# imcbrearty/GENIE

Hardware: AMD Instinct MI355X
Metric: picks/sec through GCN_Detection_Network_extended.forward_fixed_source (GCS_Network.forward) (higher is better)
Workload: dtype f32

## Files before the change

genie_amd/csrc/genie_hip.hip:

```cpp
#include <hip/hip_runtime.h>
#include <stdint.h>
#include <stdio.h>
#include <stdlib.h>
#include <string.h>

#include <algorithm>
#include <array>
#include <map>
#include <memory>
#include <mutex>
#include <utility>
#include <type_traits>
#include <string>
#include <vector>

#include "genie_hip.h"

#define GENIE_LD_STREAM(ptr) (*(ptr))
#define GENIE_S2_WAVES 2
#define GENIE_H2_DEPTH 6

namespace {

typedef float f32x4 __attribute__((ext_vector_type(4)));

thread_local std::string g_err;

int fail(int code, const std::string& msg) {
    g_err = msg;
    return code;
}

#define HIP_TRY(expr)                                                                              \
    do {                                                                                           \
        hipError_t e_ = (expr);                                                                    \
        if (e_ != hipSuccess)                                                                      \
            return fail(GENIE_ERR_HIP, std::string(#expr) + ": " + hipGetErrorString(e_));         \
    } while (0)
#define GENIE_TRY(expr)                                                                            \
    do {                                                                                           \
        if (int rc_ = (expr)) return rc_;                                                          \
    } while (0)

struct DevPool {
    std::multimap<size_t, void*> free_;
    size_t cached = 0;
};
std::map<int, DevPool> g_pools;
std::map<void*, std::pair<int, size_t>> g_pool_blocks;
std::mutex g_pool_mutex;
constexpr size_t POOL_CAP = (size_t)3 << 30;

size_t pool_class(size_t n) {
    if (n < 256) return 256;
    int sh = 0;
    while ((n >> sh) >= 16) ++sh;
    const size_t step = (size_t)1 << sh;
    return (n + step - 1) / step * step;
}

hipError_t gmalloc(void** p, size_t bytes) {
    int dev = 0;
    hipError_t e = hipGetDevice(&dev);
    if (e != hipSuccess) return e;
    const size_t cls = pool_class(bytes);
    {
        std::lock_guard<std::mutex> lk(g_pool_mutex);
        DevPool& P = g_pools[dev];
        auto it = P.free_.find(cls);
        if (it != P.free_.end()) {
            *p = it->second;
            P.cached -= cls;
            P.free_.erase(it);
            return hipSuccess;
        }
    }
    e = hipMalloc(p, cls);
    if (e != hipSuccess) {
        std::lock_guard<std::mutex> lk(g_pool_mutex);
        DevPool& P = g_pools[dev];
        (void)hipDeviceSynchronize();
        for (auto& kv : P.free_) { g_pool_blocks.erase(kv.second); (void)hipFree(kv.second); }
        P.free_.clear(); P.cached = 0;
        e = hipMalloc(p, cls);
        if (e != hipSuccess) return e;
    }
    std::lock_guard<std::mutex> lk(g_pool_mutex);
    g_pool_blocks[*p] = std::make_pair(dev, cls);
    return hipSuccess;
}
template <typename T> hipError_t gmalloc(T** p, size_t bytes) { return gmalloc((void**)p, bytes); }

hipError_t gfree(void* p) {
    if (!p) return hipSuccess;
    std::lock_guard<std::mutex> lk(g_pool_mutex);
    auto it = g_pool_blocks.find(p);
    if (it == g_pool_blocks.end()) return hipFree(p);
    DevPool& P = g_pools[it->second.first];
    const size_t cls = it->second.second;
// ... 976 lines not shown
#include "aux_kernels.hpp"
#include "train_tail_kernels.hpp"
#include "train_assoc_kernels.hpp"
#include "train_arrival_kernels.hpp"
#include "detect_kernels.hpp"
#include "stack_kernels.hpp"
#include "select_kernels.hpp"
#include "cloud_kernels.hpp"
#include "optim_kernels.hpp"
#include "pointer_kernels.hpp"

}

enum class RowLayout { Rows, NodePlanar };

struct ModelTables {
    StagePlan plan[NPLAN];
    DevBuf<StepDesc> d_steps[NPLAN];
    DevBuf<BiasDesc> d_bias[NPLAN];
    DevBuf<int32_t> d_scal[NPLAN];
    DevBuf<AccDesc> d_acc[NTM]; DevBuf<VecDesc> d_vec[NTM]; DevBuf<int32_t> d_sc[NTM];
    int n_acc[NTM] = {}, n_vec[NTM] = {}, n_sc[NTM] = {};
    DevBuf<int32_t> d_h2tbl;
    DevBuf<int32_t> d_s2htbl;
};

struct RevGraph {
    DevBuf<int32_t> rowptr, col;
    DevBuf<float> w;
    DevBuf<int2> cw;
};

struct genie_ctx {
    int S, G, G_ext, T;
    float scale_rel, scale_t;
    long long P, P_ext, E_src;
    DevBuf<int32_t> sta_rowptr, sta_col, src_rowptr, src_col, order, outdeg;
    DevBuf<float> raw;
    bool dirty;
    const ModelTables* tb;
    DevBuf<PackPlan> d_packplans; int pack_blocks;
    DevBuf<float> packed[NPLAN];
    DevBuf<float> as_pg;
    DevBuf<float> as_ps;
    RevGraph r_sta, r_src;
    RevGraph rp_sta, rp_src;
    DevBuf<int32_t> ptile16, ptile32;
    const float *xs_slice, *xs_mask;
    const void* xs_ws;
    int xs_mm_copy;
    DevBuf<float> abs_sta, abs_src;
    DevBuf<unsigned> abs_ts, abs_tg;
    bool abs_dirty;
    int abs_ts_order;
    bool pcsr;
    bool pcsr_h2;
    DevBuf<int32_t> p_sta_rowptr, p_sta_col, p_src_rowptr, p_src_col, seg_rowptr;
    DevBuf<int32_t> p_src_of;
    DevBuf<int32_t> p_sta_of;
    DevBuf<float> mpos_sta, mpos_src, ebias_sta, ebias_src;
    bool has_edges;
    DevBuf<int32_t> sta_perm, sta_inv, sta_rowptr_p, sta_col_p;
    DevBuf<int32_t> sta_ident;
    DevBuf<float> ebias_sta_p;
    const float* ea_user;
    DevBuf<int32_t> src_tab;
    DevBuf<float> packed_h2;
    hipStream_t side_stream;
    hipEvent_t ev_fork, ev_join;
    int device = 0;
    int num_cu;
    int seg, bpc1, bpc2;
    int ks_uni, kp_uni;
    int use_fast;
    int bpc2o;
    int s2_wgmap;
    int bpc1b;
    int use_h2;
    int prec_mode;
    bool range_ok;
    float range_act, range_w;
    DevBuf<float> d_range; float* h_range;
    unsigned* h_inflag;
    struct S2uTables { DevBuf<S2uBlock> blocks; DevBuf<int32_t> xcd0; int nblk; };
    std::map<std::pair<int, int>, S2uTables> s2u;
    std::vector<int32_t> tab_host;
    DevBuf<float> packed_s2h;
    DevBuf<unsigned> ea_frag, ea_frag_tmp;
    RowLayout s1_layout;
    std::vector<const void*> lds_attr_done;
    int xs_sta_order;
    int sign_input;
    int no_phase;
    int tail_f32;
    size_t o_xs, o_mm, o_c, o_wu, o_wv, o_part, o_sa0, o_sa1, o_bip, o_gpart, o_pj0, o_pj1, o_cv, ws_floats;
    size_t slot_stride;
    size_t big_stride;
    int tail_cu_ro, tail_cu_sa;
    int slot;

    ~genie_ctx() {
        if (h_range) (void)hipHostFree(h_range);
        if (h_inflag) (void)hipHostFree(h_inflag);
        if (ev_fork) (void)hipEventDestroy(ev_fork);
        if (ev_join) (void)hipEventDestroy(ev_join);
    }
};

namespace {

int raise_lds_limit(genie_ctx* c, const void* kern, int bytes) {
    for (const void* k : c->lds_attr_done) if (k == kern) return GENIE_OK;
    HIP_TRY(hipFuncSetAttribute(kern, hipFuncAttributeMaxDynamicSharedMemorySize, bytes));
    c->lds_attr_done.push_back(kern);
    return GENIE_OK;
}

long long edge_rows_sta(const genie_ctx* c) { return c->pcsr ? c->P : c->S; }
long long edge_rows_src(const genie_ctx* c) { return c->pcsr ? c->P : c->G; }
bool h2_on(const genie_ctx* c) { return c->use_h2 && (c->prec_mode == 1 || (c->prec_mode == 0 && c->range_ok)); }
bool pcsr_h2_on(const genie_ctx* c) { return c->pcsr_h2 && (c->prec_mode == 1 || (c->prec_mode == 0 && c->range_ok)); }
int part_T(const genie_ctx* c) { return c->pcsr ? 1 : c->T; }
bool abs_generic(const genie_ctx* c) { return c->abs_sta != nullptr && (c->has_edges || !h2_on(c)); }

struct StageCall {
    float* save;
    bool train;
};
constexpr StageCall kInference{nullptr, false};

bool sta_order_on(const genie_ctx* c, const StageCall& call) {
    return c->sta_perm != nullptr && !c->pcsr && h2_on(c) && !abs_generic(c) && !call.train;
}
bool tail_wide(const genie_ctx* c, const StageCall& call) { return !c->tail_f32 && !call.train; }

enum class S1Route {
    Generic,
    PcsrH2,
    PcsrF32,
    H2,
};
enum class S2Route {
    TrainAssoc,
    TrainH2u,
    TrainOrd,
    Generic,
    PcsrPseg,
    PcsrSeg,
    AssocLast,
    H2u,
};
struct StageRoutes {
    S1Route s1;
    S2Route s2;
    RowLayout layout;
};
StageRoutes stage_routes(const genie_ctx* c, const StageCall& call, int gi_begin, int gi_end, bool no_bip, bool want_xl) {
    StageRoutes r;
    if (c->pcsr) {
        r.s1 = pcsr_h2_on(c) && !(c->abs_sta && c->has_edges) ? S1Route::PcsrH2 : S1Route::PcsrF32;
        r.s2 = !no_bip && !want_xl && !call.save ? S2Route::PcsrPseg : S2Route::PcsrSeg;
    } else {
        r.s1 = h2_on(c) && !abs_generic(c) ? S1Route::H2 : S1Route::Generic;
        const bool whole = gi_begin == 0 && gi_end == c->G;
        const bool fast = c->use_fast && !abs_generic(c);
        if (call.train) {
            if (fast && no_bip && want_xl && whole) r.s2 = S2Route::TrainAssoc;
// ... 1021 lines not shown
            }
            a.abs_ts = c->abs_ts; a.abs_tg = c->abs_tg;
        }
        launch_stage1_h2<true>(a, c->abs_sta != nullptr, c->has_edges, c->P * XROW >= (1ll << 32), grid, st);
        break;
    }
    case S1Route::PcsrF32: {
        const long long ntiles = (c->P + 15) / 16;
        a.ptile = c->ptile16;
        const long long gw = std::min<long long>((ntiles + 3) / 4, (long long)c->num_cu * c->bpc1);
        k_stage1_pcsr<<<(int)std::max<long long>(8, gw / 8 * 8), 256, 0, st>>>(a);
        break;
    }
    case S1Route::H2: {
        unsigned* xs = (unsigned*)((float*)ws + c->o_xs);
        const bool presplit = (c->xs_slice == slice && c->xs_mask == mask && c->xs_ws == ws && c->xs_sta_order == (so ? 1 : 0)) || !do_split;
        if (do_split) { c->xs_slice = c->xs_mask = nullptr; c->xs_ws = nullptr; }
        float* mmw = (float*)ws + c->o_mm + (c->slot % GENIE_NBIG) * c->big_stride;
        if (presplit && do_split && so && c->xs_mm_copy != c->slot % GENIE_NBIG) {
            HIP_TRY(hipMemcpyAsync(mmw, (const float*)ws + c->o_mm + c->xs_mm_copy * c->big_stride, sizeof(float) * (size_t)c->P_ext,
                                   hipMemcpyDeviceToDevice, st));
        }
        if (!presplit) {
            if (so && c->S <= SPLIT_G_MAXS) {
                HIP_TRY(hipFuncSetAttribute((const void*)k_split_rows_g, hipFuncAttributeMaxDynamicSharedMemorySize, SPLIT_G_MAXS * 32));
                k_split_rows_g<<<(unsigned)(c->P_ext / c->S), 256, (size_t)c->S * 32, st>>>(slice, mask, c->S, xs, c->sta_perm, mmw, c->P_ext,
                                                                                            input_limit(c), c->h_inflag);
            } else
                k_split_rows<<<(unsigned)((c->P_ext + 255) / 256), 256, 0, st>>>(slice, mask, c->P_ext, xs, so ? c->sta_perm : nullptr, c->S,
                                                                                mmw, input_limit(c), c->h_inflag);
        }
        a.xs = xs; a.packed = c->packed_h2; a.xs_plane = c->P_ext * (long long)XPC;
        a.np = r.layout == RowLayout::NodePlanar ? 1 : 0;
        const int grid = da_grid_w(c, (n_tiles + 1) / 2, c->bpc1b, H2_THREADS / 64);
        if (!n_tiles) break;
        if (c->abs_sta && (c->abs_dirty || !c->abs_ts || c->abs_ts_order != (so ? 1 : 0))) {
            if (!c->abs_ts) GENIE_TRY(alloc_abs_pieces(c, (size_t)c->S, (size_t)c->G_ext));
            k_abs_pieces<<<(c->S + 255) / 256, 256, 0, st>>>(c->abs_sta, so ? c->sta_perm : nullptr, c->S, c->abs_ts);
            k_abs_pieces<<<(c->G_ext + 255) / 256, 256, 0, st>>>(c->abs_src, nullptr, c->G_ext, c->abs_tg);
            c->abs_dirty = false; c->abs_ts_order = so ? 1 : 0;
            a.abs_ts = c->abs_ts; a.abs_tg = c->abs_tg;
        }
        launch_stage1_h2<false>(a, c->abs_sta != nullptr, c->has_edges, c->P_ext * XROW >= (1ll << 32), grid, st);
        break;
    }
    }
    HIP_TRY(hipGetLastError());
    if (dbg_tmp) {
        if (dbg_h0) k_permute_sta_rows<<<(unsigned)((c->P * 30 + 255) / 256), 256, 0, st>>>(dbg_tmp, c->P, 30, c->sta_perm, c->S, dbg_h0);
        if (dbg_h1) k_permute_sta_rows<<<(unsigned)((c->P * 60 + 255) / 256), 256, 0, st>>>(dbg_tmp + c->P * 30, c->P, 60, c->sta_perm, c->S, dbg_h1);
        HIP_TRY(hipStreamSynchronize(st));
    }
    return GENIE_OK;
}
}

int genie_da_stage1(genie_ctx* c, const float* slice, const float* mask, void* ws, void* stream) {
    if (!c) return fail(GENIE_ERR_ARG, "null context");
    return run_stage1(c, kInference, slice, mask, nullptr, nullptr, ws, stream, 0, c->G, true);
}

int genie_da_stage1_range(genie_ctx* c, const float* slice, const float* mask, int gi_begin, int gi_end, int first, void* ws,
                          void* stream) {
    if (!c) return fail(GENIE_ERR_ARG, "null context");
    return run_stage1(c, kInference, slice, mask, nullptr, nullptr, ws, stream, gi_begin, gi_end, first != 0);
}

int genie_da_stage1_debug(genie_ctx* c, const float* slice, const float* mask, float* h0_out, float* h1_out, void* ws,
                          void* stream) {
    if (!c || !h0_out || !h1_out) return fail(GENIE_ERR_ARG, "genie_da_stage1_debug: null argument");
    return run_stage1(c, kInference, slice, mask, h0_out, h1_out, ws, stream, 0, c->G, true);
}

float* genie_ws_v_ptr(const genie_ctx* c, void* ws) {
    return (c && ws) ? (float*)ws + c->o_wv + (c->slot % GENIE_NBIG) * c->big_stride : nullptr;
}
int genie_ws_v_pitch(const genie_ctx* c) { (void)c; return ROWW; }

namespace {
int get_s2u_tables(genie_ctx* c, int gb0, int ge0, const genie_ctx::S2uTables** out) {
    const auto key = std::make_pair(gb0, ge0);
    auto itf = c->s2u.find(key);
    if (itf != c->s2u.end()) { *out = &itf->second; return GENIE_OK; }
    const std::vector<int32_t>& tab = c->tab_host;
    std::vector<S2uBlock> blks;
    std::vector<int32_t> seen_blk((size_t)c->G_ext, -1), seen_at((size_t)c->G_ext, 0);
    int32_t serial = 0;
    int32_t x0[9];
    const int nxc = 8, n = ge0 - gb0;
    for (int x = 0; x < nxc; ++x) {
        x0[x] = (int32_t)blks.size();
        const int gb = gb0 + (int)((long long)n * x / nxc), ge = gb0 + (int)((long long)n * (x + 1) / nxc);
        int pos = gb;
        while (pos < ge) {
            S2uBlock b;
            memset(&b, 0, sizeof(b));
            b.gi0 = pos;
            ++serial;
            int32_t uni[S2U_UCAP + 15];
            int nuni = 0;
            while (pos < ge && b.n < S2U_NB) {
                int32_t where[15];
                const int before = nuni;
                for (int k = 0; k < 15; ++k) {
                    const int32_t nb = tab[(size_t)pos * 16 + 1 + k];
                    if (seen_blk[(size_t)nb] != serial) { seen_blk[(size_t)nb] = serial; seen_at[(size_t)nb] = nuni; uni[nuni++] = nb; }
                    where[k] = seen_at[(size_t)nb];
                }
                if (b.n > 0 && nuni > S2U_UCAP) {
                    for (int u = before; u < nuni; ++u) seen_blk[(size_t)uni[u]] = -1;
                    nuni = before;
                    break;
                }
                b.idx[b.n][0] = tab[(size_t)pos * 16];
                for (int k = 0; k < 15; ++k) b.idx[b.n][1 + k] = where[k];
                ++b.n; ++pos;
            }
            for (int e = b.n; e < S2U_NB; ++e) b.idx[e][0] = -1;
            b.U = (int32_t)nuni;
            for (int u = 0; u < 64; ++u) b.ids[u] = uni[u < nuni ? u : 0];
            blks.push_back(b);
        }
    }
    x0[nxc] = (int32_t)blks.size();
    genie_ctx::S2uTables t;
    t.nblk = (int)blks.size();
    GENIE_TRY(dev_upload(t.blocks, blks));
    GENIE_TRY(dev_upload(t.xcd0, x0, (size_t)nxc + 1));
    *out = &(c->s2u[key] = std::move(t));
    return GENIE_OK;
}

extern "C++" template <bool SAVE>
int launch_stage2_h2u(genie_ctx* c, const DaArgs& a, int gi_begin, int gi_end, bool xl, hipStream_t st) {
    const genie_ctx::S2uTables* tb = nullptr;
    if (int rc = get_s2u_tables(c, gi_begin, gi_end, &tb)) return rc;
    const size_t lds = sizeof(float) * S2H_IMG_FLOATS + (size_t)S2U_UCAP * 1024;
    const long long items = (long long)tb->nblk * c->T;
    const int grid = (int)std::max<long long>(8, std::min<long long>((long long)c->num_cu * GENIE_S2U_BPC, (items + 7) / 8 * 8) / 8 * 8);
    const bool big = c->P_ext * 128 >= (1ll << 32);
    auto launch = [&](auto kern) -> int {
        if (int r = raise_lds_limit(c, (const void*)kern, 160 * 1024)) return r;
        kern<<<grid, S2U_WPB * 64, lds, st>>>(a, tb->blocks, tb->xcd0);
        return GENIE_OK;
    };
    if (xl) return big ? launch(k_stage2_h2u<true, true, SAVE>) : launch(k_stage2_h2u<true, false, SAVE>);
    return big ? launch(k_stage2_h2u<false, true, SAVE>) : launch(k_stage2_h2u<false, false, SAVE>);
}

int run_stage2(genie_ctx* c, const StageCall& call, const float* mask, const float* edge_attr, float* x_latent_out, void* ws,
               void* stream, int gi_begin, int gi_end, const float* slope2 = nullptr, int no_bip = 0) {
    int rc = check_ws(c, ws);
    if (rc) return rc;
    if (!mask || !edge_attr) return fail(GENIE_ERR_ARG, "genie_da_stage2_partials: null argument");
    if (gi_begin < 0 || gi_end > c->G || gi_begin > gi_end) return fail(GENIE_ERR_ARG, "genie_da_stage2_partials: bad source-node range");
    if (!(gi_begin == 0 && gi_end == c->G) && c->pcsr)
        return fail(GENIE_ERR_STATE, "genie_da_stage2_partials_range: not available on an irregular product graph");
    hipStream_t st = (hipStream_t)stream;
    if ((rc = ensure_packed(c, st))) return rc;
    DaArgs a = make_da_args(c, call, (float*)ws);
    a.gi0 = gi_begin; a.G = gi_end - gi_begin;
    a.slope2 = slope2; a.no_bip = no_bip;
    const long long n_tiles = (long long)a.G * c->T;
    if (n_tiles == 0) return GENIE_OK;
    const StageRoutes r = stage_routes(c, call, gi_begin, gi_end, no_bip != 0, x_latent_out != nullptr);
    if (!no_bip && c->s1_layout != r.layout)
        return fail(GENIE_ERR_STATE, r.layout == RowLayout::NodePlanar
                                         ? "stage 2: this call's stage 2 reads c / wv node-planar, but the last stage 1 wrote them as rows"
                                         : "stage 2: this call's stage 2 reads c / wv as rows, but the last stage 1 wrote them node-planar");
    a.mask = mask; a.edge_attr = edge_attr; a.x_latent = x_latent_out; a.packed = c->packed[PL_S2];
    a.ea_int = nullptr;
    a.mm_int = (const float*)ws + c->o_mm + (c->slot % GENIE_NBIG) * c->big_stride;
    auto identity_order = [&]() -> int {
        if (!c->sta_ident) {
            std::vector<int32_t> id((size_t)c->S);
            for (int i = 0; i < c->S; ++i) id[i] = i;
            GENIE_TRY(dev_upload(c->sta_ident, id));
        }
        a.sta_user = c->sta_ident; a.wgmap = 0;
        return GENIE_OK;
    };
    switch (r.s2) {
    case S2Route::TrainAssoc:
        if ((rc = identity_order())) return rc;
        k_stage2_ord<8, 15, true, true, true><<<da_grid(c, n_tiles, c->bpc2o), 256, 0, st>>>(a);
        break;
    case S2Route::TrainH2u:
        if ((rc = identity_order())) return rc;
        a.ea_int = edge_attr; a.np = 1; a.packed = c->packed_s2h;
        if (!c->ea_frag_tmp) HIP_TRY(c->ea_frag_tmp.alloc(8 * (size_t)c->P));
        k_ea_frag<<<(unsigned)((c->P + 255) / 256), 256, 0, st>>>(edge_attr, c->P, c->S, nullptr, c->ea_frag_tmp);
        a.ea_frag = c->ea_frag_tmp;
        if ((rc = launch_stage2_h2u<true>(c, a, gi_begin, gi_end, x_latent_out != nullptr, st))) return rc;
        break;
    case S2Route::TrainOrd:
        if ((rc = identity_order())) return rc;
        a.ea_int = edge_attr;
        if (x_latent_out) k_stage2_ord<8, 15, true, false, true><<<da_grid(c, n_tiles, c->bpc2o), 256, 0, st>>>(a);
        else k_stage2_ord<8, 15, false, false, true><<<da_grid(c, n_tiles, c->bpc2o), 256, 0, st>>>(a);
        break;
    case S2Route::Generic:
        k_stage2<<<da_grid(c, n_tiles, c->bpc2), 256, 0, st>>>(a);
        break;
    case S2Route::PcsrPseg: {
        a.ptile = c->ptile16;
        const long long gs = std::min<long long>((c->G + 3) / 4, (long long)c->num_cu * c->bpc2);
        k_stage2_pseg<<<(int)std::max<long long>(8, gs / 8 * 8), 256, 0, st>>>(a, c->seg_rowptr, c->G);
        break;
    }
    case S2Route::PcsrSeg: {
        const long long ntiles = (c->P + 15) / 16;
        a.ptile = c->ptile16;
        const long long gw = std::min<long long>((ntiles + 3) / 4, (long long)c->num_cu * c->bpc2);
        k_stage2_pcsr<<<(int)std::max<long long>(8, gw / 8 * 8), 256, 0, st>>>(a);
        if (!no_bip)
            k_seg_sum32<<<(c->G * 32 + 255) / 256, 256, 0, st>>>((const float*)ws + c->o_c + (c->slot % GENIE_NBIG) * c->big_stride, c->seg_rowptr,
                                                                 c->G, (float*)ws + c->o_part + c->slot * c->slot_stride);
        break;
    }
    case S2Route::AssocLast:
        a.wgmap = 0;
        k_stage2_ord<8, 15, true, true><<<da_grid(c, n_tiles, c->bpc2o), 256, 0, st>>>(a);
        break;
    case S2Route::H2u:
        a.wgmap = c->s2_wgmap; a.np = 1; a.packed = c->packed_s2h;
        if (c->ea_frag && c->ea_user == edge_attr) a.ea_frag = c->ea_frag;
// ... 1684 lines not shown
```

genie_amd/csrc/stage_kernels.hpp:

```cpp

template <int N>
__device__ __forceinline__ void mma_blocks(f32x4 (&acc)[N], const f32x4 (&w)[N], const f32x4 x) {
#pragma unroll
    for (int r = 0; r < 4; ++r) {
#pragma unroll
        for (int k = 0; k < N; ++k) acc[k] = MFMA16(w[k][r], x[r], acc[k]);
    }
}

__device__ __forceinline__ void stage1_dense(const DaArgs& a, const f32x4* lw, const float* lbias, int lane, int q,
                                             bool valid, long long p, int g, int sc, float mq, f32x4 x0, f32x4 x1, f32x4 n1a,
                                             f32x4 n1b, f32x4 n2a, f32x4 n2b, float a1, float a21, float a22) {
    if (a.dbg_h0 != nullptr && valid) {
#pragma unroll
        for (int r = 0; r < 4; ++r) {
            a.dbg_h0[p * 30 + 4 * q + r] = x0[r];
            if (16 + 4 * q + r < 30) a.dbg_h0[p * 30 + 16 + 4 * q + r] = x1[r];
        }
    }
    f32x4 acc[4], w4[4];
#pragma unroll
    for (int k = 0; k < 4; ++k) acc[k] = *(const f32x4*)(lbias + (2 + k) * 16 + 4 * q);
    if (a.eb_sta != nullptr) {
#pragma unroll
// ... 1233 lines not shown
            }
        for (int i = t; i < 990; i += 256) { const float x = fabsf(W(RG_FC1_W)[i]); bad |= !(x <= 3.0e38f); wmax = fmaxf(wmax, x); }
    }
    if (t < 30) {
        float z = fabsf(W(RG_INIT_B)[t]);
        for (int j = 0; j < 8; ++j) z += fabsf(W(RG_INIT_W)[t * 8 + j]);
        for (int j = 0; j < 3; ++j) z += fabsf(W(RG_INIT_ABS)[t * 6 + j]) * pos_sta + fabsf(W(RG_INIT_ABS)[t * 6 + 3 + j]) * pos_src;
        H0[t] = g1(a0) * z; N1[t] = g1(s11) * z; N2[t] = g1(s12) * z;
        amax = fmaxf(fmaxf(amax, fmaxf(pos_sta, pos_src)), fmaxf(H0[t], fmaxf(N1[t], N2[t])));
    }
    __syncthreads();
    if (t < 60) {
        const int i = t % 30, hf = t / 30;
        const float* w = W(hf ? RG_L1T22_W : RG_L1T12_W) + i * 64;
        const float* n = hf ? N2 : N1;
        float z = fabsf(W(hf ? RG_L1T22_B : RG_L1T12_B)[i]) + (hf ? ebg : ebs);
        for (int j = 0; j < 30; ++j) z += fabsf(w[j]) * H0[j] + fabsf(w[30 + j]) * n[j];
        for (int j = 0; j < 4; ++j) z += fabsf(w[60 + j]);
        (hf ? H1b : H1a)[i] = g1(a1) * z;
        amax = fmaxf(amax, g1(a1) * z);
    }
    __syncthreads();
    if (t < 60) {
        const int i = t % 30, hf = t / 30;
        const float* w = W(hf ? RG_L2T21_W : RG_L2T11_W) + i * 60;
        float z = fabsf(W(hf ? RG_L2T21_B : RG_L2T11_B)[i]);
        for (int j = 0; j < 30; ++j) z += fabsf(w[j]) * H1a[j] + fabsf(w[30 + j]) * H1b[j];
        const float s = hf ? a22 : a21;
        (hf ? V : U)[i] = g1(s) * z;
        amax = fmaxf(amax, g1(s) * z);
    }
    __syncthreads();
    if (t < 30) {
        const int i = t % 15, hf = t / 15;
        const float* w = W(hf ? RG_L2T22_W : RG_L2T12_W) + i * 94;
        const float* uv = hf ? V : U;
        float z = fabsf(W(hf ? RG_L2T22_B : RG_L2T12_B)[i]) + (hf ? ebg : ebs);
        for (int j = 0; j < 30; ++j) z += fabsf(w[j]) * H1a[j] + fabsf(w[30 + j]) * H1b[j] + fabsf(w[60 + j]) * uv[j];
        for (int j = 0; j < 4; ++j) z += fabsf(w[90 + j]);
        amax = fmaxf(amax, g1(a2) * z);
    }
    bad |= !(amax <= 3.0e38f);
    const float am = blk_max256(bad ? __builtin_inff() : amax, red);
    const float wm = blk_max256(bad ? __builtin_inff() : wmax, red);
    if (t == 0) {
        a.out[0] = am; a.out[1] = wm;
        a.out[2] = (am < H2_RANGE_LIMIT && wm < H2_RANGE_LIMIT) ? 1.f : 0.f;
        a.out[3] = 0.f;
    }
}

#define MFMA16H(a, b, c) \
    __builtin_amdgcn_mfma_f32_16x16x32_f16(__builtin_bit_cast(f16x8, (a)), __builtin_bit_cast(f16x8, (b)), (c), 0, 0, 0)

__global__ void k_ea_frag(const float* __restrict__ ea, long long rows, int S, const int32_t* __restrict__ sta_user,
                          unsigned* __restrict__ out) {
    const long long p = (long long)blockIdx.x * blockDim.x + threadIdx.x;
    if (p >= rows) return;
    const long long g = p / S;
    const int s = (int)(p - g * S);
    const long long pu = g * S + (sta_user != nullptr ? sta_user[s] : s);
    const float e0 = ea[pu * 3], e1 = ea[pu * 3 + 1], e2 = ea[pu * 3 + 2];
    const unsigned a0 = cvt_pk_f16(e0, e1), b0 = cvt_pk_f16(e2, 0.f);
    const unsigned a1 = cvt_pk_f16(sub_f16_lo(e0, a0), sub_f16_hi(e1, a0)), b1 = cvt_pk_f16(sub_f16_lo(e2, b0), 0.f);
    *(u32x4*)(out + ((g * 2) * S + s) * 4) = u32x4{a0, b0, a1, b1};
    *(u32x4*)(out + ((g * 2 + 1) * S + s) * 4) = u32x4{pk_mul_f16(a0, H2_SIXTEENTH), pk_mul_f16(b0, H2_SIXTEENTH), 0u, 0u};
}

template <bool BIG>
__device__ __forceinline__ unsigned long long s2h_base(const void* b, int id, unsigned pitch) {
    const unsigned long long off = BIG ? (unsigned long long)(unsigned)id * (unsigned long long)pitch
                                       : (unsigned long long)((unsigned)id * pitch);
    unsigned long long r = (unsigned long long)b + off;
    asm volatile("" : "+s"(r));
    return r;
}

constexpr int S2U_WPB = 4;
constexpr int S2U_NB = 2 * S2U_WPB;
#define GENIE_S2U_BPC 2
#define GENIE_S2U_UCAP 64
constexpr int S2U_UCAP = GENIE_S2U_UCAP;
constexpr int S2U_NSTG = S2U_UCAP / S2U_WPB;
struct S2uBlock {
    int32_t gi0, n, U, pad;
    int32_t ids[64];
    int32_t idx[S2U_NB][16];
};

template <bool XL, bool BIG, bool SAVE = false>
__global__ __launch_bounds__(S2U_WPB * 64, GENIE_S2U_BPC) void k_stage2_h2u(DaArgs a, const S2uBlock* __restrict__ blocks, const int32_t* __restrict__ xcd_blk0) {
    constexpr int KS = 8, KP = 15;
    constexpr int NF4 = S2H_IMG_FLOATS / 4;
    extern __shared__ __attribute__((aligned(16))) f32x4 s2u_smem[];
    f32x4* lw = s2u_smem;
    char* lrows = (char*)(s2u_smem + NF4);
    for (int i = threadIdx.x; i < NF4; i += blockDim.x) lw[i] = ((const f32x4*)a.packed)[i];
    const float* lbias = (const float*)(lw + S2H_FRAGS * 64);
    int lane = threadIdx.x & 63;
    const int m = lane & 15, kg = lane >> 4;
    const int jl = lane >> 2, ql = lane & 3;
    const int wave = __builtin_amdgcn_readfirstlane(threadIdx.x >> 6);
    const int S = a.S, T = a.T;
    const int nx = (a.nxcd > 1 && gridDim.x >= (unsigned)a.nxcd && (gridDim.x % a.nxcd) == 0) ? a.nxcd : 1;
    const int xcd = blockIdx.x % nx, lb = blockIdx.x / nx, nbx = gridDim.x / nx;
    const int blk0 = nx == 1 ? xcd_blk0[0] : xcd_blk0[xcd], blk1 = nx == 1 ? xcd_blk0[a.nxcd] : xcd_blk0[xcd + 1];
    const long long n_items = (long long)(blk1 - blk0) * T;
    __syncthreads();
    if (lb >= n_items) return;
    const float a2 = a.slope2 != nullptr ? *a.slope2 : lbias[32], ab1 = lbias[33];
    typedef const __attribute__((address_space(1))) char* gbytes;
    typedef const __attribute__((address_space(1))) f32x4* grow;
    typedef const __attribute__((address_space(1))) u32x4* gfrag;
    typedef const __attribute__((address_space(1))) float* gflt;
    const unsigned plane = (unsigned)S * 16u;
    const unsigned pc = (unsigned)S * 128u, pw = (unsigned)S * 64u, pe = (unsigned)S * 32u, pm = (unsigned)S * 4u;
    const unsigned kgp = (unsigned)kg * plane, kge = (unsigned)min(kg, 1) * plane;
    const unsigned q16 = 16u * (unsigned)ql;
    const int bperm = (4 * m + kg) * 4;
    const unsigned m_T = ItemIter::recip((unsigned)T);

    long long it_last = lb;
    while (it_last + nbx < n_items) it_last += nbx;
    auto item_of = [&](long long it, int& blk, int& tb) {
        const long long itr = n_items - 1 - (it <= it_last ? it : it_last);
        unsigned rem;
        const unsigned kb = T <= 1 ? (rem = 0u, (unsigned)itr) : ItemIter::fdiv((unsigned)itr, (unsigned)T, m_T, rem);
        blk = __builtin_amdgcn_readfirstlane(blk0 + (int)kb);
        tb = __builtin_amdgcn_readfirstlane((int)rem);
    };
    f32x4 stg[S2U_NSTG];
    auto stage_issue = [&](int idl, int U, int tb) {
        const int s = tb * 16 + m, sc = s < S ? s : S - 1;
        const unsigned lo = kgp + (unsigned)sc * 16u;
#pragma unroll
        for (int i = 0; i < S2U_NSTG; ++i) {
            const int u = wave + S2U_WPB * i;
            if (u < U) {
                const unsigned long long vb = s2h_base<BIG>(a.wv, __builtin_amdgcn_readlane(idl, u), pw);
                stg[i] = *(grow)((gbytes)vb + lo);
            }
        }
    };
    auto stage_write = [&](int U) {
#pragma unroll
        for (int i = 0; i < S2U_NSTG; ++i) {
            const int u = wave + S2U_WPB * i;
            if (u < U) *(f32x4*)(lrows + (unsigned)u * 1024u + (unsigned)lane * 16u) = stg[i];
        }
    };
    struct Node { f32x4 ru[KS], c1, c2; u32x4 ea; float mq; } R;
    int sta[KS];
    auto load_sta = [&](int tb) {
        const int s = tb * 16 + jl;
        load_sta_ids<KS>(a.sta_col, s < S ? s : S - 1, sta);
    };
    auto issue = [&](int idv, int tb) {
        const int g = max(__builtin_amdgcn_readlane(idv, 0), 0);
        const int s = tb * 16 + m, sc = s < S ? s : S - 1;
        const unsigned so = (unsigned)sc * 16u;
        const unsigned lo = kgp + so;
        const unsigned long long cb = s2h_base<BIG>(a.c, g, pc);
        R.c1 = *(grow)((gbytes)cb + lo);
        R.c2 = *(grow)((gbytes)cb + (lo + 4u * plane));
        const unsigned long long mb = s2h_base<BIG>(a.mm_int, g, pm);
        R.mq = *(gflt)((gbytes)mb + (unsigned)sc * 4u);
        if (s >= S) R.mq = 0.f;
        const unsigned long long eb = s2h_base<BIG>(a.ea_frag, g, pe);
        R.ea = *(gfrag)((gbytes)eb + (kge + so));
        const unsigned long long ub = s2h_base<BIG>(a.wu, g, pw);
#pragma unroll
        for (int k = 0; k < KS; ++k) R.ru[k] = *(grow)((gbytes)ub + ((unsigned)sta[k] * 64u + q16));
    };
    auto slot = [&](long long j, int& blk, int& tb, int& b) {
        item_of(lb + (j >> 1) * nbx, blk, tb);
        b = wave + S2U_WPB * (int)(j & 1);
    };
    auto idv_at = [&](long long j) {
        int blk, tb, b;
        slot(j, blk, tb, b);
        return blocks[blk].idx[b][m];
    };
    const long long n_my_items = (n_items - lb + nbx - 1) / nbx;
    int blk_c, tb_c, blk_n, tb_n, blk_2, tb_2, dummy;
    item_of(lb, blk_c, tb_c);
    item_of(lb + nbx, blk_n, tb_n);
    int idl_c = blocks[blk_c].ids[lane], U_c = blocks[blk_c].U;
    int idl_n = blocks[blk_n].ids[lane], U_n = blocks[blk_n].U;
    stage_issue(idl_c, __builtin_amdgcn_readfirstlane(U_c), tb_c);
    int idv_c = idv_at(0), idv_n = idv_at(1);
    load_sta(tb_c);
    issue(idv_c, tb_c);
    for (long long ii = 0; ii < n_my_items; ++ii) {
        const bool has_next_item = ii + 1 < n_my_items;
        item_of(lb + (ii + 2) * nbx, blk_2, tb_2);
        const int idl_2 = blocks[blk_2].ids[lane], U_2 = blocks[blk_2].U;
        stage_write(__builtin_amdgcn_readfirstlane(U_c));
        __syncthreads();
        if (has_next_item) stage_issue(idl_n, __builtin_amdgcn_readfirstlane(U_n), tb_n);
#pragma unroll
        for (int h = 0; h < 2; ++h) {
            asm volatile("" : "+v"(lane));
            const long long j = 2 * ii + h;
            const int idv_2 = idv_at(j + 2 < 2 * n_my_items ? j + 2 : j);
            const int g_raw = __builtin_amdgcn_readlane(idv_c, 0);
            const bool live = g_raw >= 0;
            const int g_c = max(g_raw, 0);
            const int tbc = tb_c;
            const int tb_next = h == 0 ? tb_c : tb_n;
            (void)dummy;
            f32x4 n1 = {0.f, 0.f, 0.f, 0.f}, n2 = {0.f, 0.f, 0.f, 0.f};
#pragma unroll
            for (int k = 0; k < KS; ++k) n1 += R.ru[k];
#pragma unroll
            for (int k0 = 0; k0 < KP; k0 += 5) {
                f32x4 rv[5];
#pragma unroll
                for (int k = 0; k < 5; ++k)
                    rv[k] = *(const f32x4*)(lrows + (unsigned)__builtin_amdgcn_readlane(idv_c, 1 + k0 + k) * 1024u + (unsigned)lane * 16u);
#pragma unroll
                for (int k = 0; k < 5; ++k) n2 += rv[k];
            }
            f32x4 n1t;
#pragma unroll
            for (int r = 0; r < 4; ++r) {
                const float v = n1[r];
                n1t[r] = __int_as_float(__builtin_amdgcn_ds_bpermute(bperm, __float_as_int(v)));
            }
            f32x4 o1 = fma4(n1t, 1.f / (float)KS, R.c1), o2 = fma4(n2, 1.f / (float)KP, R.c2);
            const float mq = R.mq;
            const u32x4 eab = R.ea;
            const long long p_sv = SAVE ? (long long)g_c * S + a.sta_user[min(tbc * 16 + m, S - 1)] : 0;
            const bool sv_ok = SAVE && live && tbc * 16 + m < S;
            if (sv_ok) {
                *(f32x4*)(a.save + ((size_t)(SV_O + 0) * a.Pn + p_sv) * 16 + 4 * kg) = o1;
                *(f32x4*)(a.save + ((size_t)(SV_O + 1) * a.Pn + p_sv) * 16 + 4 * kg) = o2;
            }
            o1 = prelu4u(o1, a2);
            o2 = prelu4u(o2, a2);
            asm volatile("" : "+v"(o1), "+v"(o2), "+v"(idv_n));
            issue(idv_n, tb_next);
            if (h == 0) load_sta(tb_n);
            if (XL && live && tbc * 16 + m < S) {
                const int su = a.sta_user[tbc * 16 + m];
                float* xl = a.x_latent + ((long long)g_c * S + su) * 30;
#pragma unroll
                for (int r = 0; r < 4; ++r)
                    if (4 * kg + r < 15) { xl[4 * kg + r] = o1[r]; xl[15 + 4 * kg + r] = o2[r]; }
            }
            u32x4 p0, p1, p2;
            p0[0] = cvt_pk_f16(o1[0], o1[1]); p0[1] = cvt_pk_f16(o1[2], o1[3]);
            p0[2] = cvt_pk_f16(o2[0], o2[1]); p0[3] = cvt_pk_f16(o2[2], o2[3]);
            p1[0] = cvt_pk_f16(sub_f16_lo(o1[0], p0[0]), sub_f16_hi(o1[1], p0[0]));
            p1[1] = cvt_pk_f16(sub_f16_lo(o1[2], p0[1]), sub_f16_hi(o1[3], p0[1]));
            p1[2] = cvt_pk_f16(sub_f16_lo(o2[0], p0[2]), sub_f16_hi(o2[1], p0[2]));
            p1[3] = cvt_pk_f16(sub_f16_lo(o2[2], p0[3]), sub_f16_hi(o2[3], p0[3]));
#pragma unroll
            for (int d = 0; d < 4; ++d) p2[d] = pk_mul_f16(p0[d], H2_SIXTEENTH);
            f32x4 bp[2];
#pragma unroll
            for (int t = 0; t < 2; ++t) {
                bp[t] = *(const f32x4*)(lbias + 16 * t + 4 * kg);
                const f32x4 w0 = lw[(S2H_FW + 2 * t) * 64 + lane], w1 = lw[(S2H_FW + 2 * t + 1) * 64 + lane];
                const f32x4 we = lw[(S2H_FE + t) * 64 + lane];
                bp[t] = MFMA16H(w0, p1, bp[t]);
                bp[t] = MFMA16H(w1, p2, bp[t]);
                bp[t] = MFMA16H(we, eab, bp[t]);
                bp[t] = MFMA16H(w0, p0, bp[t]);
                if (sv_ok) *(f32x4*)(a.save + ((size_t)(SV_ZB + t) * a.Pn + p_sv) * 16 + 4 * kg) = bp[t];
            }
#pragma unroll
            for (int t = 0; t < 2; ++t) {
                f32x4 v = prelu4u(bp[t], ab1) * mq;
                v.x = row_sum16_tree(v.x); v.y = row_sum16_tree(v.y); v.z = row_sum16_tree(v.z); v.w = row_sum16_tree(v.w);
                if (m == 0 && live) *(f32x4*)(a.part + ((long long)g_c * T + tbc) * 32 + 16 * t + 4 * kg) = v;
            }
            idv_c = idv_n; idv_n = idv_2;
        }
        if (!has_next_item) break;
        __syncthreads();
        blk_c = blk_n; tb_c = tb_n; blk_n = blk_2; tb_n = tb_2;
        idl_c = idl_n; U_c = U_n; idl_n = idl_2; U_n = U_2;
    }
}
```

Measured before the change: 78.41 million.

## Carry staged neighbour rows across grouped stage-2 blocks to reuse LDS

```diff
diff --git a/genie_amd/csrc/genie_hip.hip b/genie_amd/csrc/genie_hip.hip
--- a/genie_amd/csrc/genie_hip.hip
+++ b/genie_amd/csrc/genie_hip.hip
@@ -15,6 +15,7 @@
 #include <vector>
 
 #include "genie_hip.h"
+#include "s2u_plan.hpp"
 
 #define GENIE_LD_STREAM(ptr) (*(ptr))
 #define GENIE_S2_WAVES 2
@@ -1157,7 +1158,7 @@
     float range_act, range_w;
     DevBuf<float> d_range; float* h_range;
     unsigned* h_inflag;
-    struct S2uTables { DevBuf<S2uBlock> blocks; DevBuf<int32_t> xcd0; int nblk; };
+    struct S2uTables { DevBuf<S2uBlock> blocks; DevBuf<int32_t> xcd0; int nblk, ngroups; };
     std::map<std::pair<int, int>, S2uTables> s2u;
     std::vector<int32_t> tab_host;
     DevBuf<float> packed_s2h;
@@ -2345,51 +2346,15 @@
     const auto key = std::make_pair(gb0, ge0);
     auto itf = c->s2u.find(key);
     if (itf != c->s2u.end()) { *out = &itf->second; return GENIE_OK; }
-    const std::vector<int32_t>& tab = c->tab_host;
-    std::vector<S2uBlock> blks;
-    std::vector<int32_t> seen_blk((size_t)c->G_ext, -1), seen_at((size_t)c->G_ext, 0);
-    int32_t serial = 0;
-    int32_t x0[9];
-    const int nxc = 8, n = ge0 - gb0;
-    for (int x = 0; x < nxc; ++x) {
-        x0[x] = (int32_t)blks.size();
-        const int gb = gb0 + (int)((long long)n * x / nxc), ge = gb0 + (int)((long long)n * (x + 1) / nxc);
-        int pos = gb;
-        while (pos < ge) {
-            S2uBlock b;
-            memset(&b, 0, sizeof(b));
-            b.gi0 = pos;
-            ++serial;
-            int32_t uni[S2U_UCAP + 15];
-            int nuni = 0;
-            while (pos < ge && b.n < S2U_NB) {
-                int32_t where[15];
-                const int before = nuni;
-                for (int k = 0; k < 15; ++k) {
-                    const int32_t nb = tab[(size_t)pos * 16 + 1 + k];
-                    if (seen_blk[(size_t)nb] != serial) { seen_blk[(size_t)nb] = serial; seen_at[(size_t)nb] = nuni; uni[nuni++] = nb; }
-                    where[k] = seen_at[(size_t)nb];
-                }
-                if (b.n > 0 && nuni > S2U_UCAP) {
-                    for (int u = before; u < nuni; ++u) seen_blk[(size_t)uni[u]] = -1;
-                    nuni = before;
-                    break;
-                }
-                b.idx[b.n][0] = tab[(size_t)pos * 16];
-                for (int k = 0; k < 15; ++k) b.idx[b.n][1 + k] = where[k];
-                ++b.n; ++pos;
-            }
-            for (int e = b.n; e < S2U_NB; ++e) b.idx[e][0] = -1;
-            b.U = (int32_t)nuni;
-            for (int u = 0; u < 64; ++u) b.ids[u] = uni[u < nuni ? u : 0];
-            blks.push_back(b);
-        }
-    }
-    x0[nxc] = (int32_t)blks.size();
+    s2u_plan::Plan plan;
+    if (!s2u_plan::build(c->tab_host.data(), c->G, c->G_ext, gb0, ge0, S2U_GROUP, plan))
+        return fail(GENIE_ERR_ARG, "stage 2: a source-neighbour index outside the context's source nodes");
     genie_ctx::S2uTables t;
-    t.nblk = (int)blks.size();
-    GENIE_TRY(dev_upload(t.blocks, blks));
-    GENIE_TRY(dev_upload(t.xcd0, x0, (size_t)nxc + 1));
+    t.nblk = (int)plan.blocks.size();
+    t.ngroups = 0;
+    for (int x = 0; x < s2u_plan::NXCD; ++x) t.ngroups += (plan.xcd0[x + 1] - plan.xcd0[x] + S2U_GROUP - 1) / S2U_GROUP;
+    GENIE_TRY(dev_upload(t.blocks, plan.blocks));
+    GENIE_TRY(dev_upload(t.xcd0, plan.xcd0, (size_t)s2u_plan::NXCD + 1));
     *out = &(c->s2u[key] = std::move(t));
     return GENIE_OK;
 }
@@ -2399,12 +2364,14 @@
     const genie_ctx::S2uTables* tb = nullptr;
     if (int rc = get_s2u_tables(c, gi_begin, gi_end, &tb)) return rc;
     const size_t lds = sizeof(float) * S2H_IMG_FLOATS + (size_t)S2U_UCAP * 1024;
-    const long long items = (long long)tb->nblk * c->T;
+    static_assert(s2u_plan::NXCD == 8, "the grid below is a multiple of 8 workgroups, one share per chunk of the plan");
+    if (a.nxcd != s2u_plan::NXCD) return fail(GENIE_ERR_STATE, "stage 2: the block table is planned for 8 XCD chunks");
+    const long long items = (long long)tb->ngroups * c->T;
     const int grid = (int)std::max<long long>(8, std::min<long long>((long long)c->num_cu * GENIE_S2U_BPC, (items + 7) / 8 * 8) / 8 * 8);
     const bool big = c->P_ext * 128 >= (1ll << 32);
     auto launch = [&](auto kern) -> int {
         if (int r = raise_lds_limit(c, (const void*)kern, 160 * 1024)) return r;
-        kern<<<grid, S2U_WPB * 64, lds, st>>>(a, tb->blocks, tb->xcd0);
+        kern<<<grid, S2U_WPB * 64, lds, st>>>(a, tb->blocks, tb->xcd0, S2U_GROUP);
         return GENIE_OK;
     };
     if (xl) return big ? launch(k_stage2_h2u<true, true, SAVE>) : launch(k_stage2_h2u<true, false, SAVE>);
diff --git a/genie_amd/csrc/s2u_plan.hpp b/genie_amd/csrc/s2u_plan.hpp
--- /dev/null
+++ b/genie_amd/csrc/s2u_plan.hpp
@@ -0,0 +1,121 @@
+#pragma once
+#include <cstdint>
+#include <cstring>
+#include <vector>
+
+namespace s2u_plan {
+
+constexpr int NB = 8;
+constexpr int UCAP = 64;
+constexpr int KP = 15;
+constexpr int NXCD = 8;
+
+struct Block {
+    int32_t gi0, n, U, nst;
+    int32_t ids[64];
+    int32_t idx[NB][16];
+    uint8_t slot[64];
+};
+
+struct Plan {
+    std::vector<Block> blocks;
+    int32_t xcd0[NXCD + 1];
+    int L;
+    long long rows_union, rows_carried;
+    double carried_fraction() const { return rows_union ? (double)rows_carried / (double)rows_union : 0.0; }
+};
+
+inline bool build(const int32_t* tab, int n_pos, int n_nodes, int gb0, int ge0, int L, Plan& out) {
+    out.blocks.clear();
+    out.L = L;
+    out.rows_union = out.rows_carried = 0;
+    for (int x = 0; x <= NXCD; ++x) out.xcd0[x] = 0;
+    if (!tab || gb0 < 0 || ge0 > n_pos || gb0 > ge0 || L < 1 || n_nodes < 1) return false;
+    for (size_t i = (size_t)gb0 * 16; i < (size_t)ge0 * 16; ++i)
+        if ((i & 15) && (tab[i] < 0 || tab[i] >= n_nodes)) return false;
+    std::vector<int32_t> seen_blk((size_t)n_nodes, -1), seen_at((size_t)n_nodes, 0);
+    std::vector<int32_t> slot_of((size_t)n_nodes, -1);
+    int32_t serial = 0;
+    const int n = ge0 - gb0;
+    for (int x = 0; x < NXCD; ++x) {
+        out.xcd0[x] = (int32_t)out.blocks.size();
+        const int gb = gb0 + (int)((long long)n * x / NXCD), ge = gb0 + (int)((long long)n * (x + 1) / NXCD);
+        int pos = gb;
+        int32_t occ[UCAP], last_use[UCAP];
+        int in_group = 0;
+        for (int s = 0; s < UCAP; ++s) { occ[s] = -1; last_use[s] = -1; }
+        while (pos < ge) {
+            Block b;
+            memset(&b, 0, sizeof(b));
+            b.gi0 = pos;
+            ++serial;
+            int32_t uni[UCAP + KP];
+            int nuni = 0;
+            while (pos < ge && b.n < NB) {
+                int32_t where[KP];
+                const int before = nuni;
+                for (int k = 0; k < KP; ++k) {
+                    const int32_t nb = tab[(size_t)pos * 16 + 1 + k];
+                    if (seen_blk[(size_t)nb] != serial) { seen_blk[(size_t)nb] = serial; seen_at[(size_t)nb] = nuni; uni[nuni++] = nb; }
+                    where[k] = seen_at[(size_t)nb];
+                }
+                if (b.n > 0 && nuni > UCAP) {
+                    for (int u = before; u < nuni; ++u) seen_blk[(size_t)uni[u]] = -1;
+                    nuni = before;
+                    break;
+                }
+                b.idx[b.n][0] = tab[(size_t)pos * 16];
+                for (int k = 0; k < KP; ++k) b.idx[b.n][1 + k] = where[k];
+                ++b.n; ++pos;
+            }
+            if (nuni > UCAP) return false;
+            for (int e = b.n; e < NB; ++e) b.idx[e][0] = -1;
+            b.U = (int32_t)nuni;
+            int32_t slot_u[UCAP];
+            int nst = 0;
+            if (in_group == 0) {
+                for (int s = 0; s < UCAP; ++s) {
+                    if (occ[s] >= 0) slot_of[(size_t)occ[s]] = -1;
+                    occ[s] = -1; last_use[s] = -1;
+                }
+                for (int u = 0; u < nuni; ++u) {
+                    slot_u[u] = u;
+                    b.ids[nst] = uni[u]; b.slot[nst] = (uint8_t)u; ++nst;
+                }
+            } else {
+                for (int u = 0; u < nuni; ++u) {
+                    slot_u[u] = slot_of[(size_t)uni[u]];
+                    if (slot_u[u] >= 0) last_use[slot_u[u]] = serial;
+                }
+                for (int u = 0; u < nuni; ++u) {
+                    if (slot_u[u] >= 0) continue;
+                    int best = -1;
+                    for (int s = 0; s < UCAP; ++s)
+                        if (last_use[s] != serial && (best < 0 || last_use[s] < last_use[best])) best = s;
+                    if (best < 0) return false;
+                    slot_u[u] = best; last_use[best] = serial;
+                    b.ids[nst] = uni[u]; b.slot[nst] = (uint8_t)best; ++nst;
+                }
+            }
+            for (int e = 0; e < nst; ++e) {
+                const int s = b.slot[e];
+                if (occ[s] >= 0) slot_of[(size_t)occ[s]] = -1;
+                occ[s] = b.ids[e]; slot_of[(size_t)b.ids[e]] = s; last_use[s] = serial;
+            }
+            b.nst = nst;
+            for (int e = nst; e < 64; ++e) b.ids[e] = nst ? b.ids[0] : uni[0];
+            for (int i = 0; i < b.n; ++i)
+                for (int k = 0; k < KP; ++k) b.idx[i][1 + k] = slot_u[b.idx[i][1 + k]];
+            out.rows_union += nuni;
+            out.rows_carried += nuni - nst;
+            out.blocks.push_back(b);
+            if (++in_group == L) in_group = 0;
+        }
+        for (int s = 0; s < UCAP; ++s)
+            if (occ[s] >= 0) slot_of[(size_t)occ[s]] = -1;
+    }
+    out.xcd0[NXCD] = (int32_t)out.blocks.size();
+    return true;
+}
+
+}
diff --git a/genie_amd/csrc/stage_kernels.hpp b/genie_amd/csrc/stage_kernels.hpp
--- a/genie_amd/csrc/stage_kernels.hpp
+++ b/genie_amd/csrc/stage_kernels.hpp
@@ -1339,14 +1339,15 @@
 #define GENIE_S2U_UCAP 64
 constexpr int S2U_UCAP = GENIE_S2U_UCAP;
 constexpr int S2U_NSTG = S2U_UCAP / S2U_WPB;
-struct S2uBlock {
-    int32_t gi0, n, U, pad;
-    int32_t ids[64];
-    int32_t idx[S2U_NB][16];
-};
+#ifndef GENIE_S2U_GROUP
+#define GENIE_S2U_GROUP 4
+#endif
+constexpr int S2U_GROUP = GENIE_S2U_GROUP;
+typedef s2u_plan::Block S2uBlock;
+static_assert(s2u_plan::NB == S2U_NB && s2u_plan::UCAP == S2U_UCAP, "s2u_plan.hpp cuts blocks for another kernel shape");
 
 template <bool XL, bool BIG, bool SAVE = false>
-__global__ __launch_bounds__(S2U_WPB * 64, GENIE_S2U_BPC) void k_stage2_h2u(DaArgs a, const S2uBlock* __restrict__ blocks, const int32_t* __restrict__ xcd_blk0) {
+__global__ __launch_bounds__(S2U_WPB * 64, GENIE_S2U_BPC) void k_stage2_h2u(DaArgs a, const S2uBlock* __restrict__ blocks, const int32_t* __restrict__ xcd_blk0, int L) {
     constexpr int KS = 8, KP = 15;
     constexpr int NF4 = S2H_IMG_FLOATS / 4;
     extern __shared__ __attribute__((aligned(16))) f32x4 s2u_smem[];
@@ -1359,10 +1360,10 @@
     const int jl = lane >> 2, ql = lane & 3;
     const int wave = __builtin_amdgcn_readfirstlane(threadIdx.x >> 6);
     const int S = a.S, T = a.T;
-    const int nx = (a.nxcd > 1 && gridDim.x >= (unsigned)a.nxcd && (gridDim.x % a.nxcd) == 0) ? a.nxcd : 1;
+    constexpr int nx = s2u_plan::NXCD;
     const int xcd = blockIdx.x % nx, lb = blockIdx.x / nx, nbx = gridDim.x / nx;
-    const int blk0 = nx == 1 ? xcd_blk0[0] : xcd_blk0[xcd], blk1 = nx == 1 ? xcd_blk0[a.nxcd] : xcd_blk0[xcd + 1];
-    const long long n_items = (long long)(blk1 - blk0) * T;
+    const int blk0 = xcd_blk0[xcd], blk1 = xcd_blk0[xcd + 1];
+    const long long n_items = (long long)((blk1 - blk0 + L - 1) / L) * T;
     __syncthreads();
     if (lb >= n_items) return;
     const float a2 = a.slope2 != nullptr ? *a.slope2 : lbias[32], ab1 = lbias[33];
@@ -1377,14 +1378,23 @@
     const int bperm = (4 * m + kg) * 4;
     const unsigned m_T = ItemIter::recip((unsigned)T);
 
-    long long it_last = lb;
-    while (it_last + nbx < n_items) it_last += nbx;
-    auto item_of = [&](long long it, int& blk, int& tb) {
-        const long long itr = n_items - 1 - (it <= it_last ? it : it_last);
+    struct Cur { long long it; int blk, end, tb; };
+    auto item_at = [&](long long it) {
+        const long long itr = n_items - 1 - it;
         unsigned rem;
         const unsigned kb = T <= 1 ? (rem = 0u, (unsigned)itr) : ItemIter::fdiv((unsigned)itr, (unsigned)T, m_T, rem);
-        blk = __builtin_amdgcn_readfirstlane(blk0 + (int)kb);
-        tb = __builtin_amdgcn_readfirstlane((int)rem);
+        Cur c;
+        c.it = it;
+        c.blk = __builtin_amdgcn_readfirstlane(blk0 + (int)kb * L);
+        c.end = min(c.blk + L, blk1);
+        c.tb = __builtin_amdgcn_readfirstlane((int)rem);
+        return c;
+    };
+    auto step = [&](Cur& c) {
+        if (c.blk + 1 < c.end) { ++c.blk; return true; }
+        if (c.it + nbx >= n_items) return false;
+        c = item_at(c.it + nbx);
+        return true;
     };
     f32x4 stg[S2U_NSTG];
     auto stage_issue = [&](int idl, int U, int tb) {
@@ -1399,11 +1409,11 @@
             }
         }
     };
-    auto stage_write = [&](int U) {
+    auto stage_write = [&](int sll, int U) {
 #pragma unroll
         for (int i = 0; i < S2U_NSTG; ++i) {
             const int u = wave + S2U_WPB * i;
-            if (u < U) *(f32x4*)(lrows + (unsigned)u * 1024u + (unsigned)lane * 16u) = stg[i];
+            if (u < U) *(f32x4*)(lrows + (unsigned)__builtin_amdgcn_readlane(sll, u) * 1024u + (unsigned)lane * 16u) = stg[i];
         }
     };
     struct Node { f32x4 ru[KS], c1, c2; u32x4 ea; float mq; } R;
@@ -1429,43 +1439,33 @@
 #pragma unroll
         for (int k = 0; k < KS; ++k) R.ru[k] = *(grow)((gbytes)ub + ((unsigned)sta[k] * 64u + q16));
     };
-    auto slot = [&](long long j, int& blk, int& tb, int& b) {
-        item_of(lb + (j >> 1) * nbx, blk, tb);
-        b = wave + S2U_WPB * (int)(j & 1);
-    };
-    auto idv_at = [&](long long j) {
-        int blk, tb, b;
-        slot(j, blk, tb, b);
-        return blocks[blk].idx[b][m];
-    };
-    const long long n_my_items = (n_items - lb + nbx - 1) / nbx;
-    int blk_c, tb_c, blk_n, tb_n, blk_2, tb_2, dummy;
-    item_of(lb, blk_c, tb_c);
-    item_of(lb + nbx, blk_n, tb_n);
-    int idl_c = blocks[blk_c].ids[lane], U_c = blocks[blk_c].U;
-    int idl_n = blocks[blk_n].ids[lane], U_n = blocks[blk_n].U;
+    Cur cc = item_at(lb), cn = cc;
+    bool has_next = step(cn);
+    Cur c2 = cn;
+    bool has_2 = step(c2);
+    int blk_c = cc.blk, tb_c = cc.tb, blk_n = cn.blk, tb_n = cn.tb;
+    int idl_c = blocks[blk_c].ids[lane], sll_c = blocks[blk_c].slot[lane], U_c = blocks[blk_c].nst;
+    int idl_n = blocks[blk_n].ids[lane], sll_n = blocks[blk_n].slot[lane], U_n = blocks[blk_n].nst;
     stage_issue(idl_c, __builtin_amdgcn_readfirstlane(U_c), tb_c);
-    int idv_c = idv_at(0), idv_n = idv_at(1);
+    int idv_c = blocks[blk_c].idx[wave][m], idv_n = blocks[blk_c].idx[wave + S2U_WPB][m];
     load_sta(tb_c);
     issue(idv_c, tb_c);
-    for (long long ii = 0; ii < n_my_items; ++ii) {
-        const bool has_next_item = ii + 1 < n_my_items;
-        item_of(lb + (ii + 2) * nbx, blk_2, tb_2);
-        const int idl_2 = blocks[blk_2].ids[lane], U_2 = blocks[blk_2].U;
-        stage_write(__builtin_amdgcn_readfirstlane(U_c));
+    for (;;) {
+        const bool has_next_item = has_next;
+        const int blk_2 = c2.blk, tb_2 = c2.tb;
+        const int idl_2 = blocks[blk_2].ids[lane], sll_2 = blocks[blk_2].slot[lane], U_2 = blocks[blk_2].nst;
+        stage_write(sll_c, __builtin_amdgcn_readfirstlane(U_c));
         __syncthreads();
         if (has_next_item) stage_issue(idl_n, __builtin_amdgcn_readfirstlane(U_n), tb_n);
 #pragma unroll
         for (int h = 0; h < 2; ++h) {
             asm volatile("" : "+v"(lane));
-            const long long j = 2 * ii + h;
-            const int idv_2 = idv_at(j + 2 < 2 * n_my_items ? j + 2 : j);
+            const int idv_2 = blocks[blk_n].idx[wave + S2U_WPB * h][m];
             const int g_raw = __builtin_amdgcn_readlane(idv_c, 0);
             const bool live = g_raw >= 0;
             const int g_c = max(g_raw, 0);
             const int tbc = tb_c;
             const int tb_next = h == 0 ? tb_c : tb_n;
-            (void)dummy;
             f32x4 n1 = {0.f, 0.f, 0.f, 0.f}, n2 = {0.f, 0.f, 0.f, 0.f};
 #pragma unroll
             for (int k = 0; k < KS; ++k) n1 += R.ru[k];
@@ -1537,6 +1537,8 @@
         if (!has_next_item) break;
         __syncthreads();
         blk_c = blk_n; tb_c = tb_n; blk_n = blk_2; tb_n = tb_2;
-        idl_c = idl_n; U_c = U_n; idl_n = idl_2; U_n = U_2;
-    }
-}
+        idl_c = idl_n; sll_c = sll_n; U_c = U_n; idl_n = idl_2; sll_n = sll_2; U_n = U_2;
+        has_next = has_2;
+        has_2 = step(c2);
+    }
+}
```

Result: faster. 79.89 million (median of 6 runs) (+1.9%).
